# gabrielmittag/NISQA

Hardware: AMD Instinct MI355X
Metric: clips/sec (10 s, 48 kHz) (higher is better)
Workload: dtype bf16x6 (every GEMM -- CNN, projection, self-attention, pooling: fp32 operands as three exact bf16 terms, 6 MFMA products per term pair, f32 accumulate: all 24 operand mantissa bits; mel f32)

## Files before the change

include/nisqa_hip.h:

```cpp
#ifndef NISQA_HIP_H
#define NISQA_HIP_H

#include <stddef.h>
#include <stdint.h>

#ifdef __cplusplus
extern "C" {
#endif

#define NISQA_OK 0
#define NISQA_ERR_ARG 1
#define NISQA_ERR_LAUNCH 2
#define NISQA_ERR_WORKSPACE 3

#define NISQA_ABI_VERSION 2
#define NISQA_N_MELS 48
#define NISQA_SEG_LEN 15
#define NISQA_N_FFT 4096
#define NISQA_FEAT 384
#define NISQA_DMODEL 64

int nisqa_abi_version(void);

typedef struct {
// ... 151 lines not shown
    const uint16_t* pool_wb;
    int32_t arch;
} nisqa_model_dev;

size_t nisqa_workspace_bytes(int32_t n_clips, int32_t total_frames, int32_t total_tok_padded);

int nisqa_predict_batch(const float* pcm, const int64_t* clip_off, const int32_t* frame_off,
                        const int32_t* tok_off, const int32_t* n_wins, int32_t n_clips,
                        int32_t total_frames, int32_t total_tok_padded,
                        const nisqa_mel_cfg* cfg, const nisqa_model_dev* model,
                        void* ws, size_t ws_bytes, float* out, void* stream);

int nisqa_predict_batch_pcm16(const int16_t* pcm, const int64_t* clip_off, const int32_t* frame_off,
                              const int32_t* tok_off, const int32_t* n_wins, int32_t n_clips,
                              int32_t total_frames, int32_t total_tok_padded,
                              const nisqa_mel_cfg* cfg, const nisqa_model_dev* model,
                              void* ws, size_t ws_bytes, float* out, void* stream);

int nisqa_pcm16_to_f32(const int16_t* pcm16, float* pcm, int64_t n, void* stream);

#define NISQA_WAVENC_PCM 1
#define NISQA_WAVENC_FLOAT 3
#define NISQA_WAVENC_ALAW 6
#define NISQA_WAVENC_MULAW 7
#define NISQA_WAVENC_BIG_ENDIAN 0x10000
typedef struct nisqa_wav_clip {
    int64_t src_off;
    int64_t dst_off;
    int64_t n_frames;
    int32_t channels;
    int32_t container;
    int32_t encoding;
    int32_t channel;
} nisqa_wav_clip;
int nisqa_wav_decode(const void* raw, int64_t raw_bytes, const nisqa_wav_clip* clips, int32_t n_clips,
                     int64_t max_frames, float* out, void* stream);

#define NISQA_FLAC_BAD_MD5 0x80
#define NISQA_FLAC_BAD_TABLE 0x100
typedef struct nisqa_flac_clip {
    int64_t src_off;
    int64_t src_bytes;
    int64_t dst_off;
    int64_t n_samples;
    int64_t md5_off;
    int32_t frame0;
    int32_t n_frames;
    int32_t block_size;
    int32_t bits;
    int32_t channels;
    int32_t channel;
    int32_t md5_set;
    int32_t reserved;
    uint8_t md5[16];
} nisqa_flac_clip;
#ifndef NISQA_FLAC_FRAME_DEFINED
#define NISQA_FLAC_FRAME_DEFINED
typedef struct nisqa_flac_frame {
    int32_t offset;
    int32_t first_sample;
    int32_t block_size;
    int32_t clip;
} nisqa_flac_frame;
#endif
size_t nisqa_flac_workspace_bytes(int32_t n_frames, int32_t max_block, int32_t max_channels, int64_t md5_bytes);
int nisqa_flac_decode(const void* raw, int64_t raw_bytes, const nisqa_flac_clip* clips, int32_t n_clips,
                      const nisqa_flac_frame* frames, int32_t n_frames, int32_t max_block, int32_t max_channels,
                      int32_t out_i16, void* out, int64_t out_samples, int64_t md5_bytes, void* ws, size_t ws_bytes,
                      int32_t* status, void* stream);

size_t nisqa_resample_workspace_bytes(int32_t n_clips, int64_t max_out);
int nisqa_resample(const void* pcm, int32_t is_pcm16, const int64_t* in_off, const int64_t* out_off, const int64_t* out_valid,
                   int32_t n_clips, int64_t max_out, double ratio, const float* table, int32_t nwin, int32_t num_table,
                   void* ws, size_t ws_bytes, float* out, void* stream);

int nisqa_de_align_fuse(const float* x, const int32_t* deg_tok_off, const int32_t* deg_n_wins, const int32_t* ref_tok_off,
                        const int32_t* ref_n_wins, int32_t n_pairs, int32_t total_deg_tok_padded, int32_t align, int32_t apply,
                        int32_t fuse, int32_t ld_out, float* out, int32_t* idx_out, void* stream);

int nisqa_selftest_mfma(const float* a, const float* b, float* d, int32_t k, void* stream);

int nisqa_probe_mfma_sustained(const void* operands, float* out, uint64_t* clk, int32_t blocks, int32_t iters, void* stream);

#ifdef __cplusplus
}
#endif
#endif
```

nisqa_amd/csrc/cnn_bf16.hip:

```cpp
#include "common.hpp"
#include "layout.hpp"
#include <stdlib.h>
#include <atomic>
#include "conv_bf16.hpp"
#include "internal.hpp"
#include "../../include/nisqa_hip.h"
#define NQ_RING2 3
#define NQ_RING34 3

#define FB_RS1 48
#define FB_P1 (168 * FB_RS1)
#define FB_RS2 80
#define FB_P2 (60 * FB_RS2)
#define FB_RS3 144
#define FB_P3 (60 * FB_RS3)
#define FB_PS (72 * FB_RS3)
#define FB_PATCH(T) ((T) * FB_P1)
#define FB_PPLANE 1700
#define FB_ZADDR 2048u
#define FB_BASE 2176u
#define FB_WAVE(T) (((T) * (FB_P1 + FB_PPLANE) + 63u) / 64u * 64u)
#define FB_WGS(T) ((T) == 2 ? 2 : 1)
#define FB_LDS(T) (FB_BASE + 4 * FB_WAVE(T))
static_assert(FB_WAVE(2) == 19584 && FB_LDS(2) == 80512 && 2 * FB_LDS(2) <= 160 * 1024, "two terms: two workgroups (8 waves) per CU");
static_assert(FB_WAVE(3) == 29312 && FB_LDS(3) == 119424 && FB_LDS(3) <= 160 * 1024 && 2 * FB_LDS(3) > 160 * 1024, "three terms: one workgroup per CU");
#define FB_PLAN_OK(T) (FB_PATCH(T) + (T) * FB_PPLANE <= FB_WAVE(T) && (T) * FB_P3 <= FB_WAVE(T) && (T) * FB_PS <= 2 * FB_WAVE(T))
static_assert(FB_PLAN_OK(2) && FB_PLAN_OK(3), "LDS plan");

__device__ constexpr int bwin75_lo(int b) { return b == 0 ? 0 : b == 1 ? 1 : b == 2 ? 2 : b == 3 ? 4 : 5; }
__device__ constexpr int bwin75_hi(int b) { return b == 0 ? 2 : b == 1 ? 3 : b == 2 ? 5 : b == 3 ? 6 : 7; }
__device__ constexpr int bwin53_lo(int b) { return b == 0 ? 0 : b == 1 ? 1 : 3; }
__device__ constexpr int bwin53_hi(int b) { return b == 0 ? 2 : b == 1 ? 4 : 5; }

NQ_CLK_EXPORT(g_phase_clk, nisqa_debug_phase_clock)
NQ_CLK_EXPORT(g_phase_clk6, nisqa_debug_phase_clock6)

#define FB_TAB5 0u
#define FB_TAB6 1024u
NQ_DEV f32x2_t lds_ld64(unsigned a) { return *(NQ_AS3 const f32x2_t*)(a); }
template <int FMT>
NQ_DEV float epi_fmt(float v, float c, float t) {
    return FMT == NQ_FMT_BF16X3 || FMT == NQ_FMT_BF16X6 ? fmaxf(v + t, 0.f) : fmaxf(fmaf(v, c, t), 0.f);
}

template <int FMT, int CIN, int MT, int NT, int W, int RS, int PLANE, bool APF, int RING>
NQ_DEV void fb_conv_k(f32x16 (&acc)[MT][NT], __amdgpu_buffer_rsrc_t wrs, int wbyte, unsigned lane16, const unsigned (&base)[MT],
                      const unsigned (&m9)[MT], conv_k_ring<FMT == NQ_FMT_BF16X6 ? 3 : 2, NT, 3>& ring) {
    if constexpr (FMT == NQ_FMT_BF16X6) conv_k_terms_ring<3, CIN, MT, NT, W, RS, PLANE, FB_ZADDR, 3, true, true>(acc, wrs, wbyte, lane16, base, m9, ring);
    else conv_k_bf16<CIN, MT, NT, W, RS, PLANE, FB_ZADDR, APF, RING, FMT>(acc, wrs, wbyte, lane16, base, m9);
}

template <int FMT, bool SEGX, bool P3>
NQ_DEV void cnn_front_split_body(
    const float* __restrict__ mel_tm, const int32_t* __restrict__ frame_off,
    const int32_t* __restrict__ tok_off, const int32_t* __restrict__ n_wins,
    const float* __restrict__ clip_floor, int n_clips, int seg_hop,
    const float* __restrict__ cw, const unsigned short* __restrict__ wb, float* __restrict__ p3,
    float* __restrict__ feat, const float* __restrict__ seg_x, int seg_L,
    const uint32_t* __restrict__ clip_max_enc, float top_db) {
    extern __shared__ __attribute__((aligned(16))) char smem[];
    constexpr bool X6 = FMT == NQ_FMT_BF16X6, F16 = FMT == NQ_FMT_F16X3 || FMT == NQ_FMT_F16X4;
    constexpr int T = X6 ? 3 : 2;
    constexpr bool T16_3 = X6 && (NQ_T16 & 1), T16_4 = X6 && (NQ_T16 & 2);
    constexpr bool CP1 = X6 && (NQ_CPAIR & 1), CP2 = X6 && (NQ_CPAIR & 2);
    static_assert(!P3 || FMT == NQ_FMT_BF16X3, "the fp32 copy of the pooled conv4 tensor is a bf16x3 debug output");
    constexpr int W1_ = X6 ? CNNX_W1 : CNNB_W1, W2_ = X6 ? CNNX_W2 : CNNB_W2, W3_ = X6 ? CNNX_W3 : CNNB_W3, W4_ = X6 ? CNNX_W4 : CNNB_W4,
                  W5_ = X6 ? CNNX_W5 : CNNB_W5, W6_ = X6 ? CNNX_W6 : CNNB_W6, WU16_ = X6 ? CNNX_U16S : CNNB_U16S;
    const int* __restrict__ meta_i = (const int*)(wb + CNNH_META);
    const float* __restrict__ meta_f = (const float*)(wb + CNNH_META);
    float dummy_mx = 0.f;
    NQ_STAMP_BEGIN();
    const int lane = threadIdx.x & 63;
    const int wave = __builtin_amdgcn_readfirstlane(threadIdx.x >> 6);
    const int p0 = blockIdx.x * 4;
    const int b = __builtin_amdgcn_readfirstlane(find_segment_wave(tok_off, n_clips, p0, lane));
    const int k0 = p0 - tok_off[b];
    const int nvalid = min(4, n_wins[b] - k0);
    if (nvalid <= 0) return;
    const bool valid = wave < nvalid;
    const int p = p0 + wave, k = k0 + wave;
    const unsigned R = FB_BASE + wave * FB_WAVE(T);
    const unsigned lane16 = lane * 16;
    const __amdgpu_buffer_rsrc_t wrs = __builtin_amdgcn_make_buffer_rsrc((void*)wb, 0, WU16_ * 2, 0x00020000);
    NQ_STAMP(0);

    const float fl = SEGX ? -3.0e38f : clip_max_enc ? dec_ordered(clip_max_enc[b]) - top_db : clip_floor[b];
    const float* src = SEGX ? seg_x + ((size_t)b * seg_L + k) * 720
                            : mel_tm + (size_t)(frame_off[b] + k * seg_hop) * 48;
    float vraw[12];
#pragma unroll
    for (int q = 0; q < 12; ++q) {
        const int i0 = lane + 64 * q;
        vraw[q] = (valid && (q < 11 || lane < 16)) ? src[i0] : 0.f;
    }
    const float tn1 = cw[CNN_T1 + (lane & 15)], tn2 = cw[CNN_T2 + (lane & 31)];
    const float tn3[2] = {cw[CNN_T3 + (lane & 31)], cw[CNN_T3 + 32 + (lane & 31)]};
    const float tn4[2] = {cw[CNN_T4 + (lane & 31)], cw[CNN_T4 + 32 + (lane & 31)]};
    const float tn5 = cw[CNN_T5 + 16 * wave + (lane & 15)], tn6 = cw[CNN_T6 + 16 * wave + (lane & 15)];
    float vin[12];
#pragma unroll
    for (int q = 0; q < 12; ++q) vin[q] = !valid ? 0.f : SEGX ? vraw[q] : fmaxf(vraw[q], fl);
    int e_in = 0;
    float m_in = 0.f;
    float s0 = 1.f;
    if (F16) {
        float mr = 0.f;
#pragma unroll
        for (int q = 0; q < 12; ++q) mr = fmaxf(mr, __builtin_fabsf(vin[q]));
        m_in = wave_max_nonneg(mr);
        e_in = f16_scale_exp(m_in);
        s0 = pow2_f32(e_in);
    }
    {
        const unsigned pb = R + FB_PATCH(T);
        constexpr int NZ = (T * FB_PPLANE + 15) / 16;
#pragma unroll
        for (int it = 0; it < (NZ + 63) / 64; ++it)
            if (64 * it + 64 <= NZ || lane < NZ - 64 * it) lds_st128(pb + (lane + 64 * it) * 16, f32x4{0.f, 0.f, 0.f, 0.f});
        if (lane < 32) ((unsigned*)(smem + FB_ZADDR))[lane] = 0u;
        __builtin_amdgcn_wave_barrier();
        if (!SEGX) {
            unsigned ob[3];
#pragma unroll
            for (int u = 0; u < 3; ++u) {
                const int e = lane + 16 * u, j0 = e >= 48 ? 1 : 0, m = e - 48 * j0;
                ob[u] = pb + ((j0 + 1) * 50 + m + 1) * 2;
            }
#pragma unroll
            for (int q = 0; q < 12; q += 2) {
                const float v0 = vin[q] * s0, v1 = vin[q + 1] * s0;
                lds_store_pair_fmt<FMT>(ob[q % 3] + (q + q / 3) * 100, ob[(q + 1) % 3] + (q + 1 + (q + 1) / 3) * 100, FB_PPLANE, v0, v1,
                                               dummy_mx, true, q + 1 < 11 || lane < 16);
            }
        } else {
#pragma unroll
            for (int q = 0; q < 12; ++q) {
                const int i0 = lane + 64 * q;
                const int m = i0 / 15, j = i0 - 15 * m;
                if (i0 < 720) lds_store_one_fmt<FMT>(pb + ((j + 1) * 50 + (m + 1)) * 2, FB_PPLANE, vin[q] * s0, dummy_mx);
            }
        }
    }
    __builtin_amdgcn_wave_barrier();
    NQ_STAMP(1);

    const int i = lane & 31, hfi = (i >> 2) & 1, qi = (i & 3) + 4 * (i >> 3);
    const int n = lane & 31, hf = lane >> 5, h = lane >> 5;
    const bool odd = (lane & 1) != 0;

    conv_k_ring<T, 1, 3> ring2;
    if constexpr (X6) conv_k_preload(ring2, wrs, W2_ * 2, lane16);
    {
        f32x4 w1[1][T];
#pragma unroll
        for (int t = 0; t < T; ++t) w1[0][t] = wfrag_load(wrs, lane16, (W1_ + t * 512) * 2);
        float tn = tn1, c1 = 1.f, ms1 = 0.f;
        int e1 = 0;
// ... 396 lines not shown
#pragma unroll
            for (int q = 0; q < T; ++q) b6[g][q] = wfrag_load(wrs, lane16, w6b + (g * T + q) * 1024);
        {
            const unsigned wr = S5 + (4 * kg) * FB_RS3 + ch * 2;
#pragma unroll
            for (int t = 0; t < 5; ++t)
#pragma unroll
                for (int r = 0; r < 4; r += 2)
                    if (t < 4 || kg < 2) {
                        f32x2_t cs0 = {1.f, 1.f}, cs1 = {1.f, 1.f};
                        if (F16) { cs0 = lds_ld64(FB_TAB5 + (16 * t + r) * 8 + kg * 32); cs1 = lds_ld64(FB_TAB5 + (16 * t + r + 1) * 8 + kg * 32); }
                        lds_store_pair_fmt<FMT>(wr + (16 * t + r) * FB_RS3, wr + (16 * t + r + 1) * FB_RS3, FB_PS,
                                                epi_fmt<FMT>(acc5[t][r], cs0[0], tn5 * cs0[1]), epi_fmt<FMT>(acc5[t][r + 1], cs1[0], tn5 * cs1[1]), dummy_mx);
                    }
        }
        __syncthreads();
        NQ_STAMP(10);

        f32x4 acc6[2], acc6b[2];
        unsigned base6[2], m6[2];
#pragma unroll
        for (int t = 0; t < 2; ++t) {
            acc6[t] = f32x4{0.f, 0.f, 0.f, 0.f};
            acc6b[t] = acc6[t];
            const int rho = 16 * t + i16;
            const int slot = rho / 6, y = rho - 6 * slot;
            m6[t] = tap_mask(rho < 24, y, 1, 6, 3);
            base6[t] = S5 + (slot * 18 + (y - 1) * 3) * FB_RS3 + (kg << 4);
        }
        unsigned a6ad[2][T];
        f32x4 a6[2][2][T];
        auto load_a6 = [&](int g) {
            const int tap = g >> 1, s = g & 1;
            const int tapoff = ((tap / 3) * 3 + tap % 3) * FB_RS3;
            if (s == 0) {
#pragma unroll
                for (int t = 0; t < 2; ++t) {
                    const bool ok = (m6[t] >> tap) & 1u;
#pragma unroll
                    for (int q = 0; q < T; ++q) a6ad[t][q] = ok ? base6[t] + q * FB_PS : FB_ZADDR - tapoff;
                }
            }
#pragma unroll
            for (int t = 0; t < 2; ++t)
#pragma unroll
                for (int q = 0; q < T; ++q) a6[g & 1][t][q] = lds_ld128(a6ad[t][q] + tapoff + 64 * s);
        };
        load_a6(0);
#pragma unroll
        for (int g = 0; g < 18; ++g) {
            if (g + 7 < 18) {
#pragma unroll
                for (int q = 0; q < T; ++q) b6[(g + 7) & 7][q] = wfrag_load(wrs, lane16, w6b + ((g + 7) * T + q) * 1024);
            }
            if (g + 1 < 18) load_a6(g + 1);
            f32x4 (&acc)[2] = (g & 1) ? acc6b : acc6;
            if constexpr (X6) {
                __builtin_amdgcn_sched_barrier(0);
                mma16_terms<T, 2>(acc, a6[g & 1], b6[g & 7]);
            } else mma16_pair_fmt<FMT, 2>(acc, a6[g & 1], b6[g & 7]);
        }
        NQ_STAMP(11);
        const unsigned fo = S4 + wave * 2048;
#pragma unroll
        for (int t = 0; t < 2; ++t)
#pragma unroll
            for (int r = 0; r < 4; ++r) {
                const int rho = 16 * t + 4 * kg + r;
                const int slot = rho / 6, y = rho - 6 * slot;
                if (rho < 24) {
                    const float c6 = F16 ? __uint_as_float(lds_ld32(FB_TAB6 + (16 * t + r) * 4 + kg * 16)) : 1.f;
                    lds_st32(fo + (slot * 96 + i16 * 6 + y) * 4, __float_as_uint(epi_fmt<FMT>(acc6[t][r] + acc6b[t][r], c6, tn6)));
                }
            }
        __builtin_amdgcn_wave_barrier();
#pragma unroll
        for (int q0 = 0; q0 < 96; q0 += 64) {
            const int q = q0 + lane;
            const int slot = q / 24;
            if (q < 96 && slot < nvalid)
                *(f32x4*)(feat + (size_t)(p0 + slot) * 384 + 96 * wave + 4 * (q - 24 * slot)) = lds_ld128(fo + 16 * q);
        }
    }
    NQ_STAMP_END((X6 ? g_phase_clk6 : g_phase_clk), ((blockIdx.y * gridDim.x + blockIdx.x) << 2) + wave);
}

#define FB_PARAMS                                                                                                              \
    const float* __restrict__ mel_tm, const int32_t* __restrict__ frame_off, const int32_t* __restrict__ tok_off,             \
    const int32_t* __restrict__ n_wins, const float* __restrict__ clip_floor, int n_clips, int seg_hop,                       \
    const float* __restrict__ cw, const unsigned short* __restrict__ wb, float* __restrict__ p3, float* __restrict__ feat,    \
    const float* __restrict__ seg_x, int seg_L, const uint32_t* __restrict__ clip_max_enc, float top_db
#define FB_ARGS mel_tm, frame_off, tok_off, n_wins, clip_floor, n_clips, seg_hop, cw, wb, p3, feat, seg_x, seg_L, clip_max_enc, top_db
template <bool SEGX, bool P3>
__global__ __launch_bounds__(256, FB_WGS(2)) void cnn_front_bf16_kernel(FB_PARAMS) {
    cnn_front_split_body<NQ_FMT_BF16X3, SEGX, P3>(FB_ARGS);
}
template <bool P4, bool SEGX>
__global__ __launch_bounds__(256, FB_WGS(2)) void cnn_front_f16_kernel(FB_PARAMS) {
    cnn_front_split_body<P4 ? NQ_FMT_F16X4 : NQ_FMT_F16X3, SEGX, false>(FB_ARGS);
}
template <bool SEGX>
__global__ __launch_bounds__(256, FB_WGS(3)) void cnn_front_bf16x6_kernel(FB_PARAMS) {
    cnn_front_split_body<NQ_FMT_BF16X6, SEGX, false>(FB_ARGS);
}

typedef void (*fb_kernel_t)(const float*, const int32_t*, const int32_t*, const int32_t*, const float*, int, int, const float*,
                            const unsigned short*, float*, float*, const float*, int, const uint32_t*, float);
static int fb_launch(int fmt, bool segx, bool p3, const float* mel_tm, const int32_t* frame_off, const int32_t* tok_off,
                     const int32_t* n_wins, const float* clip_floor, const uint32_t* clip_max_enc, float top_db, int32_t n_clips,
                     int32_t total_tok_padded, int32_t seg_hop, const float* cnn_w, const uint16_t* cnn_wb, float* p3_opt, float* feat,
                     const float* seg_x, int32_t seg_L, void* stream) {
    if (n_clips <= 0 || total_tok_padded <= 0 || (total_tok_padded & 31) || seg_hop <= 0 || !cnn_wb || !feat || fmt < 0 || fmt > 3 ||
        (p3 && fmt != 0) || (segx && (!seg_x || seg_L <= 0)) || (!segx && !clip_floor && !clip_max_enc))
        return NISQA_ERR_ARG;
    static const fb_kernel_t kernels[9] = {
        cnn_front_bf16_kernel<false, false>, cnn_front_bf16_kernel<false, true>, cnn_front_bf16_kernel<true, false>,
        cnn_front_f16_kernel<false, false>, cnn_front_f16_kernel<false, true>, cnn_front_f16_kernel<true, false>, cnn_front_f16_kernel<true, true>,
        cnn_front_bf16x6_kernel<false>, cnn_front_bf16x6_kernel<true>};
    const int which = fmt == 0 ? (segx ? 2 : p3 ? 1 : 0) : 3 + 2 * (fmt - 1) + (segx ? 1 : 0);
    const unsigned lds = fmt == NQ_FMT_BF16X6 ? FB_LDS(3) : FB_LDS(2);
    NQ_LAUNCH_BEGIN();
    static std::atomic<bool> lds_ok[9][64];
    if (nq_lds_opt_in((const void*)kernels[which], (int)lds, lds_ok[which])) return 2;
    hipLaunchKernelGGL(kernels[which], dim3(total_tok_padded / 4), dim3(256), lds, (hipStream_t)stream, mel_tm, frame_off, tok_off, n_wins,
                       clip_floor, n_clips, seg_hop, cnn_w, cnn_wb, p3_opt, feat, seg_x, seg_L, clip_max_enc, top_db);
    return NQ_LAUNCH_STATUS();
}

extern "C" int nisqa_cnn_adapt_bf16(const float* mel_tm, const int32_t* frame_off, const int32_t* tok_off,
                                    const int32_t* n_wins, const float* clip_floor, int32_t n_clips,
                                    int32_t total_tok_padded, int32_t seg_hop, const float* cnn_w,
                                    const uint16_t* cnn_wb, float* p3_opt, float* feat, void* stream) {
    if (!clip_floor) return NISQA_ERR_ARG;
    return fb_launch(0, false, p3_opt != nullptr, mel_tm, frame_off, tok_off, n_wins, clip_floor, nullptr, 0.f, n_clips, total_tok_padded, seg_hop,
                     cnn_w, cnn_wb, p3_opt, feat, nullptr, 0, stream);
}

int nq_cnn_adapt_bf16_from_max(const float* mel_tm, const int32_t* frame_off, const int32_t* tok_off,
                               const int32_t* n_wins, const uint32_t* clip_max_enc, float top_db, int32_t n_clips,
                               int32_t total_tok_padded, int32_t seg_hop, const float* cnn_w, const uint16_t* cnn_wb,
                               float* feat, void* stream) {
    if (!clip_max_enc) return NISQA_ERR_ARG;
    return fb_launch(0, false, false, mel_tm, frame_off, tok_off, n_wins, nullptr, clip_max_enc, top_db, n_clips, total_tok_padded, seg_hop, cnn_w,
                     cnn_wb, nullptr, feat, nullptr, 0, stream);
}

extern "C" int nisqa_cnn_adapt_segments_bf16(const float* x, int32_t seg_len_padded, const int32_t* tok_off,
                                             const int32_t* n_wins, int32_t n_clips, int32_t total_tok_padded,
                                             const float* cnn_w, const uint16_t* cnn_wb, float* feat, void* stream) {
    return fb_launch(0, true, false, nullptr, nullptr, tok_off, n_wins, nullptr, nullptr, 0.f, n_clips, total_tok_padded, 1, cnn_w, cnn_wb, nullptr,
                     feat, x, seg_len_padded, stream);
}

extern "C" int nisqa_cnn_adapt_f16(const float* mel_tm, const int32_t* frame_off, const int32_t* tok_off, const int32_t* n_wins,
                                   const float* clip_floor, int32_t n_clips, int32_t total_tok_padded, int32_t seg_hop,
                                   const float* cnn_w, const uint16_t* cnn_wh, int32_t products, float* feat, void* stream) {
    if (!clip_floor || (products != 3 && products != 4)) return NISQA_ERR_ARG;
    return fb_launch(products - 2, false, false, mel_tm, frame_off, tok_off, n_wins, clip_floor, nullptr, 0.f, n_clips, total_tok_padded, seg_hop,
                     cnn_w, cnn_wh, nullptr, feat, nullptr, 0, stream);
}
int nq_cnn_adapt_f16_from_max(const float* mel_tm, const int32_t* frame_off, const int32_t* tok_off, const int32_t* n_wins,
                              const uint32_t* clip_max_enc, float top_db, int32_t n_clips, int32_t total_tok_padded, int32_t seg_hop,
                              const float* cnn_w, const uint16_t* cnn_wh, int32_t products, float* feat, void* stream) {
    if (!clip_max_enc || (products != 3 && products != 4)) return NISQA_ERR_ARG;
    return fb_launch(products - 2, false, false, mel_tm, frame_off, tok_off, n_wins, nullptr, clip_max_enc, top_db, n_clips, total_tok_padded,
                     seg_hop, cnn_w, cnn_wh, nullptr, feat, nullptr, 0, stream);
}
extern "C" int nisqa_cnn_adapt_segments_f16(const float* x, int32_t seg_len_padded, const int32_t* tok_off, const int32_t* n_wins,
                                            int32_t n_clips, int32_t total_tok_padded, const float* cnn_w, const uint16_t* cnn_wh,
                                            int32_t products, float* feat, void* stream) {
    if (products != 3 && products != 4) return NISQA_ERR_ARG;
    return fb_launch(products - 2, true, false, nullptr, nullptr, tok_off, n_wins, nullptr, nullptr, 0.f, n_clips, total_tok_padded, 1, cnn_w, cnn_wh,
                     nullptr, feat, x, seg_len_padded, stream);
}

extern "C" int nisqa_cnn_adapt_bf16x6(const float* mel_tm, const int32_t* frame_off, const int32_t* tok_off,
                                      const int32_t* n_wins, const float* clip_floor, int32_t n_clips,
                                      int32_t total_tok_padded, int32_t seg_hop, const float* cnn_w,
                                      const uint16_t* cnn_wx, float* feat, void* stream) {
    return fb_launch(NQ_FMT_BF16X6, false, false, mel_tm, frame_off, tok_off, n_wins, clip_floor, nullptr, 0.f, n_clips, total_tok_padded, seg_hop,
                     cnn_w, cnn_wx, nullptr, feat, nullptr, 0, stream);
}
int nq_cnn_adapt_bf16x6_from_max(const float* mel_tm, const int32_t* frame_off, const int32_t* tok_off,
                                 const int32_t* n_wins, const uint32_t* clip_max_enc, float top_db, int32_t n_clips,
                                 int32_t total_tok_padded, int32_t seg_hop, const float* cnn_w, const uint16_t* cnn_wx,
                                 float* feat, void* stream) {
    if (!clip_max_enc) return NISQA_ERR_ARG;
    return fb_launch(NQ_FMT_BF16X6, false, false, mel_tm, frame_off, tok_off, n_wins, nullptr, clip_max_enc, top_db, n_clips, total_tok_padded,
                     seg_hop, cnn_w, cnn_wx, nullptr, feat, nullptr, 0, stream);
}
extern "C" int nisqa_cnn_adapt_segments_bf16x6(const float* x, int32_t seg_len_padded, const int32_t* tok_off,
                                               const int32_t* n_wins, int32_t n_clips, int32_t total_tok_padded,
                                               const float* cnn_w, const uint16_t* cnn_wx, float* feat, void* stream) {
    return fb_launch(NQ_FMT_BF16X6, true, false, nullptr, nullptr, tok_off, n_wins, nullptr, nullptr, 0.f, n_clips, total_tok_padded, 1, cnn_w, cnn_wx,
                     nullptr, feat, x, seg_len_padded, stream);
}
```

nisqa_amd/csrc/internal.hpp:

```cpp
#pragma once
#include <stdint.h>

int nq_cnn_adapt_bf16_from_max(const float* mel_tm, const int32_t* frame_off, const int32_t* tok_off,
                               const int32_t* n_wins, const uint32_t* clip_max_enc, float top_db, int32_t n_clips,
                               int32_t total_tok_padded, int32_t seg_hop, const float* cnn_w, const uint16_t* cnn_wb,
                               float* feat, void* stream);

int nq_cnn_adapt_f16_from_max(const float* mel_tm, const int32_t* frame_off, const int32_t* tok_off, const int32_t* n_wins,
                              const uint32_t* clip_max_enc, float top_db, int32_t n_clips, int32_t total_tok_padded, int32_t seg_hop,
                              const float* cnn_w, const uint16_t* cnn_wh, int32_t products, float* feat, void* stream);

int nq_cnn_adapt_bf16x6_from_max(const float* mel_tm, const int32_t* frame_off, const int32_t* tok_off,
                                 const int32_t* n_wins, const uint32_t* clip_max_enc, float top_db, int32_t n_clips,
                                 int32_t total_tok_padded, int32_t seg_hop, const float* cnn_w, const uint16_t* cnn_wx,
                                 float* feat, void* stream);
```

nisqa_amd/lib.py:

```python
import ctypes
import os

_HERE = os.path.dirname(os.path.abspath(__file__))
LIB_PATH = os.environ.get('NISQA_HIP_LIB') or os.path.join(_HERE, 'libnisqa_hip.so')

NISQA_OK, NISQA_ERR_ARG, NISQA_ERR_LAUNCH, NISQA_ERR_WORKSPACE = 0, 1, 2, 3
ABI_VERSION = 2
LSTM_POOL_LAST_STEP_BI, LSTM_POOL_AVG, LSTM_POOL_MAX = 0, 1, 2

c_p = ctypes.c_void_p
c_i32 = ctypes.c_int32
c_i64 = ctypes.c_int64


class MelCfg(ctypes.Structure):
    _fields_ = [('n_fft', c_i32), ('hop', c_i32), ('win', c_i32), ('n_mels', c_i32), ('n_bins', c_i32),
                ('w_floats', c_i32), ('amin_sq', ctypes.c_float), ('top_db', ctypes.c_float)]


class ModelDev(ctypes.Structure):
    _fields_ = [('window', c_p), ('twiddle', c_p), ('band_start', c_p), ('band_len', c_p), ('band_woff', c_p),
                ('band_w', c_p), ('cnn_w', c_p), ('td_w', c_p), ('pool_w', c_p),
                ('n_layers', c_i32), ('n_heads', c_i32), ('seg_hop', c_i32), ('stage_events', c_p),
                ('cnn_wb', c_p), ('cnn_mode', c_i32), ('td_wb', c_p), ('pool_wb', c_p), ('arch', c_i32)]


class WavClip(ctypes.Structure):
    _fields_ = [('src_off', c_i64), ('dst_off', c_i64), ('n_frames', c_i64), ('channels', c_i32), ('container', c_i32),
                ('encoding', c_i32), ('channel', c_i32)]


class FlacClip(ctypes.Structure):
    _fields_ = [('src_off', c_i64), ('src_bytes', c_i64), ('dst_off', c_i64), ('n_samples', c_i64), ('md5_off', c_i64),
                ('frame0', c_i32), ('n_frames', c_i32), ('block_size', c_i32), ('bits', c_i32), ('channels', c_i32),
                ('channel', c_i32), ('md5_set', c_i32), ('reserved', c_i32), ('md5', ctypes.c_uint8 * 16)]


class FlacFrame(ctypes.Structure):
    _fields_ = [('offset', c_i32), ('first_sample', c_i32), ('block_size', c_i32), ('clip', c_i32)]


FLAC_BAD_MD5, FLAC_BAD_TABLE = 0x80, 0x100
WAVENC_PCM, WAVENC_FLOAT, WAVENC_ALAW, WAVENC_MULAW, WAVENC_BIG_ENDIAN = 1, 3, 6, 7, 0x10000
MEL_GATHER_LDS_CLIPS = 1024
WAV_DECODE_MAX_BLOCK, WAV_DECODE_MAX_MEAN = 1024, 32

SYMBOLS = {
    'nisqa_abi_version': (ctypes.c_int, []),
    'nisqa_mel_db': (ctypes.c_int, [c_p, c_p, c_p, c_i32, c_i32, ctypes.POINTER(MelCfg), c_p, c_p, c_p, c_p, c_p, c_p,
                                    c_p, c_p, c_p]),
    'nisqa_mel_db_pcm16': (ctypes.c_int, [c_p, c_p, c_p, c_i32, c_i32, ctypes.POINTER(MelCfg), c_p, c_p, c_p, c_p, c_p, c_p,
                                          c_p, c_p, c_p]),
    'nisqa_mel_finalize': (ctypes.c_int, [c_p, c_p, c_i32, c_i32, c_p, ctypes.c_float, c_p, c_i32, c_p]),
    'nisqa_cnn_adapt': (ctypes.c_int, [c_p, c_p, c_p, c_p, c_p, c_i32, c_i32, c_i32, c_p, c_p, c_p, c_p]),
    'nisqa_cnn_front': (ctypes.c_int, [c_p, c_p, c_p, c_p, c_p, c_i32, c_i32, c_i32, c_p, c_p, c_p]),
    'nisqa_cnn_adapt_bf16': (ctypes.c_int, [c_p, c_p, c_p, c_p, c_p, c_i32, c_i32, c_i32, c_p, c_p, c_p, c_p, c_p]),
    'nisqa_cnn_adapt_segments_bf16': (ctypes.c_int, [c_p, c_i32, c_p, c_p, c_i32, c_i32, c_p, c_p, c_p, c_p]),
    'nisqa_cnn_adapt_bf16x6': (ctypes.c_int, [c_p, c_p, c_p, c_p, c_p, c_i32, c_i32, c_i32, c_p, c_p, c_p, c_p]),
    'nisqa_cnn_adapt_segments_bf16x6': (ctypes.c_int, [c_p, c_i32, c_p, c_p, c_i32, c_i32, c_p, c_p, c_p, c_p]),
    'nisqa_cnn_adapt_f16': (ctypes.c_int, [c_p, c_p, c_p, c_p, c_p, c_i32, c_i32, c_i32, c_p, c_p, c_i32, c_p, c_p]),
    'nisqa_cnn_adapt_segments_f16': (ctypes.c_int, [c_p, c_i32, c_p, c_p, c_i32, c_i32, c_p, c_p, c_i32, c_p, c_p]),
    'nisqa_cnn_adapt_segments': (ctypes.c_int, [c_p, c_i32, c_p, c_p, c_i32, c_i32, c_p, c_p, c_p, c_p]),
    'nisqa_cnn_back': (ctypes.c_int, [c_p, c_p, c_p, c_i32, c_i32, c_p, c_p, c_p]),
    'nisqa_cnn_standard': (ctypes.c_int, [c_p, c_p, c_p, c_p, c_p, c_i32, c_i32, c_i32, c_p, c_p, c_p, c_p]),
    'nisqa_cnn_standard_bf16': (ctypes.c_int, [c_p, c_p, c_p, c_p, c_p, c_i32, c_i32, c_i32, c_p, c_p, c_p, c_p]),
    'nisqa_cnn_standard_bf16x6': (ctypes.c_int, [c_p, c_p, c_p, c_p, c_p, c_i32, c_i32, c_i32, c_p, c_p, c_p, c_p]),
    'nisqa_cnn_standard_f16': (ctypes.c_int, [c_p, c_p, c_p, c_p, c_p, c_i32, c_i32, c_i32, c_p, c_p, c_i32, c_p, c_p]),
    'nisqa_cnn_standard_segments': (ctypes.c_int, [c_p, c_i32, c_p, c_p, c_i32, c_i32, c_p, c_p, c_p, c_p]),
    'nisqa_cnn_standard_segments_bf16': (ctypes.c_int, [c_p, c_i32, c_p, c_p, c_i32, c_i32, c_p, c_p, c_p, c_p]),
    'nisqa_cnn_standard_segments_bf16x6': (ctypes.c_int, [c_p, c_i32, c_p, c_p, c_i32, c_i32, c_p, c_p, c_p, c_p]),
    'nisqa_cnn_standard_segments_f16': (ctypes.c_int, [c_p, c_i32, c_p, c_p, c_i32, c_i32, c_p, c_p, c_i32, c_p, c_p]),
    'nisqa_lstm_laststep': (ctypes.c_int, [c_p, c_p, c_p, c_i32, c_p, c_p, c_p, c_p, c_p]),
    'nisqa_lstm_pool': (ctypes.c_int, [c_p, c_p, c_p, c_i32, c_p, c_i32, c_p, c_p, c_p, c_p]),
    'nisqa_td_selfatt': (ctypes.c_int, [c_p, c_p, c_p, c_i32, c_i32, c_i32, c_p, c_p, c_p, c_p]),
    'nisqa_td_selfatt_bf16': (ctypes.c_int, [c_p, c_p, c_p, c_i32, c_i32, c_i32, c_p, c_p, c_p, c_p, c_p]),
    'nisqa_pool_att_bf16': (ctypes.c_int, [c_p, c_p, c_p, c_i32, c_i32, c_i32, c_p, c_p, c_p, c_p, c_p]),
    'nisqa_td_selfatt_bf16x6': (ctypes.c_int, [c_p, c_p, c_p, c_i32, c_i32, c_i32, c_p, c_p, c_p, c_p, c_p]),
    'nisqa_pool_att_bf16x6': (ctypes.c_int, [c_p, c_p, c_p, c_i32, c_i32, c_i32, c_p, c_p, c_p, c_p, c_p]),
    'nisqa_td_pool_bf16x6': (ctypes.c_int, [c_p, c_p, c_p, c_i32, c_i32, c_i32, c_p, c_p, c_i32, c_p, c_p, c_p, c_p, c_p, c_p]),
    'nisqa_pool_score_bf16': (ctypes.c_int, [c_p, c_p, c_p, c_i32, c_i32, c_i32, c_p, c_p, c_p, c_p]),
    'nisqa_pool_score_bf16x6': (ctypes.c_int, [c_p, c_p, c_p, c_i32, c_i32, c_i32, c_p, c_p, c_p, c_p]),
    'nisqa_pool_final': (ctypes.c_int, [c_p, c_p, c_i32, c_i32, c_i32, c_p, c_p, c_p]),
    'nisqa_pool_att': (ctypes.c_int, [c_p, c_p, c_p, c_i32, c_i32, c_i32, c_p, c_p, c_p, c_p]),
    'nisqa_pool_profile': (ctypes.c_int, [c_p, c_i32, c_p, c_p, c_i32, c_i32, c_i32, c_i32, c_p, c_p, c_p, c_p]),
    'nisqa_pool_profile_bwd': (ctypes.c_int, [c_p, c_i32, c_p, c_p, c_i32, c_i32, c_i32, c_i32, c_p, c_p, c_p, c_p, c_p, c_p]),
    'nisqa_workspace_bytes': (ctypes.c_size_t, [c_i32, c_i32, c_i32]),
    'nisqa_predict_batch': (ctypes.c_int, [c_p, c_p, c_p, c_p, c_p, c_i32, c_i32, c_i32, ctypes.POINTER(MelCfg),
                                           ctypes.POINTER(ModelDev), c_p, ctypes.c_size_t, c_p, c_p]),
    'nisqa_predict_batch_pcm16': (ctypes.c_int, [c_p, c_p, c_p, c_p, c_p, c_i32, c_i32, c_i32, ctypes.POINTER(MelCfg),
                                                 ctypes.POINTER(ModelDev), c_p, ctypes.c_size_t, c_p, c_p]),
    'nisqa_pcm16_to_f32': (ctypes.c_int, [c_p, c_p, c_i64, c_p]),
    'nisqa_wav_decode': (ctypes.c_int, [c_p, c_i64, c_p, c_i32, c_i64, c_p, c_p]),
    'nisqa_flac_workspace_bytes': (ctypes.c_size_t, [c_i32, c_i32, c_i32, c_i64]),
    'nisqa_flac_decode': (ctypes.c_int, [c_p, c_i64, c_p, c_i32, c_p, c_i32, c_i32, c_i32, c_i32, c_p, c_i64, c_i64, c_p,
                                         ctypes.c_size_t, c_p, c_p]),
    'nisqa_resample_workspace_bytes': (ctypes.c_size_t, [c_i32, c_i64]),
    'nisqa_resample': (ctypes.c_int, [c_p, c_i32, c_p, c_p, c_p, c_i32, c_i64, ctypes.c_double, c_p, c_i32, c_i32, c_p, ctypes.c_size_t, c_p, c_p]),
    'nisqa_de_align_fuse': (ctypes.c_int, [c_p, c_p, c_p, c_p, c_p, c_i32, c_i32, c_i32, c_i32, c_i32, c_i32, c_p, c_p, c_p]),
    'nisqa_selftest_mfma': (ctypes.c_int, [c_p, c_p, c_p, c_i32, c_p]),
    'nisqa_probe_mfma_sustained': (ctypes.c_int, [c_p, c_p, c_p, c_i32, c_i32, c_p]),
}

class TdTrainArgs(ctypes.Structure):
    _fields_ = [('n_clips', c_i32), ('n_tokens', c_i32), ('n_tokens_padded', c_i32), ('n_layers', c_i32), ('n_heads', c_i32),
                ('n_wgrad_groups', c_i32), ('n_wgrad_tiles', c_i32), ('n_colsum_jobs', c_i32),
                ('seg_off', c_p), ('ptok_off', c_p), ('tile_clip', c_p), ('sq_off', c_p), ('params', c_p), ('grads', c_p),
                ('poff', c_p), ('ws', c_p), ('frags', c_p), ('labels', c_p), ('bias_map', c_p), ('inv_count', c_p),
                ('mask_p', c_p * 4), ('mask_1', c_p * 4), ('mask_f', c_p * 4), ('mask_2', c_p * 4),
                ('wgrad_desc', c_p), ('colsum_jobs', c_p)]


c_f = ctypes.c_float
TRAIN_SYMBOLS = {
    'nisqa_tdtrain_plan': (ctypes.c_int, [c_i32, c_i32, c_i32, c_i32, c_i32, c_p, c_p, c_i64]),
    'nisqa_tdtrain_step': (ctypes.c_int, [ctypes.POINTER(TdTrainArgs), c_p]),
    'nisqa_tdtrain_step_heads': (ctypes.c_int, [ctypes.POINTER(TdTrainArgs), c_p]),
    'nisqa_gemm_f32': (ctypes.c_int, [c_p, c_p, c_p, c_p, c_i32, c_i32, c_i32, c_i32, c_i32, c_f, c_p]),
    'nisqa_gemm_f32_one': (ctypes.c_int, [c_p, c_p, c_p, c_i64, c_i64, c_i64, c_i64, c_i64, c_i64, c_i32, c_i32, c_i32,
                                          c_f, c_p, c_i32, c_p]),
    'nisqa_gemm_f32_one_tile': (ctypes.c_int, [c_i64, c_i64, ctypes.POINTER(c_i32), ctypes.POINTER(c_i32)]),
    'nisqa_conv1_fwd': (ctypes.c_int, [c_p, c_p, c_p, c_p, c_i32, c_i32, c_i32, c_p, c_p, c_p, c_p]),
    'nisqa_conv1_wgrad': (ctypes.c_int, [c_p, c_p, c_p, c_p, c_i32, c_i32, c_i32, c_p, c_p, c_p]),
    'nisqa_conv1_moments': (ctypes.c_int, [c_p, c_p, c_p, c_p, c_i32, c_i32, c_i32, c_p, c_p]),
    'nisqa_conv1_bn_act_pool_fwd': (ctypes.c_int, [c_p] * 4 + [c_i32] * 3 + [c_p] * 13),
    'nisqa_conv1_bn_act_pool_bwd': (ctypes.c_int, [c_p] * 4 + [c_i32] * 3 + [c_p] * 14),
    'nisqa_im2col_mel': (ctypes.c_int, [c_p, c_p, c_p, c_p, c_i32, c_i32, c_i32, c_p, c_p]),
    'nisqa_conv1_bn_act_pool_std_fwd': (ctypes.c_int, [c_p] * 4 + [c_i32] * 3 + [c_p] * 13),
    'nisqa_conv1_bn_act_pool_std_bwd': (ctypes.c_int, [c_p] * 4 + [c_i32] * 3 + [c_p] * 14),
    'nisqa_lstm_train_fwd': (ctypes.c_int, [c_p, c_p, c_i32, c_p, c_p, c_p, c_p, c_i32, c_p, c_p, c_p, c_p, c_p]),
    'nisqa_lstm_train_bptt': (ctypes.c_int, [c_p, c_i32, c_p, c_p, c_i32, c_p, c_p, c_p, c_p, c_p]),
    'nisqa_im2col3x3': (ctypes.c_int, [c_p, c_i32, c_i32, c_i32, c_i32, c_i32, c_p, c_p]),
    'nisqa_conv3x3_gemm': (ctypes.c_int, [c_i32, c_p, c_p, c_p, c_i32, c_i32, c_i32, c_i32, c_i32, c_i32, c_p, c_i32, c_p]),
    'nisqa_conv3x3_fwd_stats': (ctypes.c_int, [c_i32, c_p, c_p, c_p, c_i32, c_i32, c_i32, c_i32, c_i32, c_i32, c_p, c_p, c_p]),
    'nisqa_conv3x3_gemm_bf16': (ctypes.c_int, [c_i32, c_p, c_p, c_p, c_i32, c_i32, c_i32, c_i32, c_i32, c_i32, c_p, c_i32, c_p]),
    'nisqa_segconv_supported': (ctypes.c_int, [c_i32, c_i32, c_i32, c_i32, c_i32]),
    'nisqa_segconv_frag_bytes': (ctypes.c_int64, [c_i32, c_i32, c_i32]),
    'nisqa_segconv_pack': (ctypes.c_int, [c_i32, c_p, c_i32, c_i32, c_p, c_p]),
    'nisqa_segconv_pack_many': (ctypes.c_int, [c_i32, c_p, c_p, c_p, c_p, c_p, c_p]),
    'nisqa_segconv_bf16': (ctypes.c_int, [c_i32, c_p, c_p, c_p, c_i32, c_i32, c_i32, c_i32, c_i32, c_i32, c_p, c_p, c_p]),
    'nisqa_segconv_frag_bytes_f32': (ctypes.c_int64, [c_i32, c_i32, c_i32]),
    'nisqa_segconv_pack_f32_many': (ctypes.c_int, [c_i32, c_p, c_p, c_p, c_p, c_p, c_p]),
    'nisqa_segconv_f32': (ctypes.c_int, [c_i32, c_p, c_p, c_p, c_i32, c_i32, c_i32, c_i32, c_i32, c_i32, c_p, c_p, c_p]),
    'nisqa_segconv_frag_bytes_x6': (ctypes.c_int64, [c_i32, c_i32, c_i32]),
    'nisqa_segconv_frag_bytes_f16': (ctypes.c_int64, [c_i32, c_i32, c_i32]),
    'nisqa_segconv_pack_f16_many': (ctypes.c_int, [c_i32, c_p, c_p, c_p, c_p, c_p, c_p]),
    'nisqa_segconv_f16': (ctypes.c_int, [c_i32, c_p, c_p, c_p, c_i32, c_i32, c_i32, c_i32, c_i32, c_i32, c_p, c_p, c_p]),
    'nisqa_segconv_pack_x6_many': (ctypes.c_int, [c_i32, c_p, c_p, c_p, c_p, c_p, c_p]),
    'nisqa_segconv_bf16x6': (ctypes.c_int, [c_i32, c_p, c_p, c_p, c_i32, c_i32, c_i32, c_i32, c_i32, c_i32, c_p, c_p, c_p]),
    'nisqa_segconv_wgrad_bf16': (ctypes.c_int, [c_p, c_p, c_p, c_i32, c_i32, c_i32, c_i32, c_i32, c_i32, c_p]),
    'nisqa_col2im3x3': (ctypes.c_int, [c_p, c_i32, c_i32, c_i32, c_i32, c_i32, c_p, c_p]),
    'nisqa_col_dot': (ctypes.c_int, [c_p, c_p, c_i64, c_i32, c_p, c_p]),
    'nisqa_bn_act_pool_fwd': (ctypes.c_int, [c_p, c_p, c_p, c_p, c_p, c_p, c_p, c_i32, c_i32, c_i32, c_i32, c_i32, c_i32,
                                             c_p, c_p, c_p, c_p]),
    'nisqa_bn_act_pool_bwd1': (ctypes.c_int, [c_p, c_p, c_p, c_p, c_p, c_p, c_p, c_i32, c_i32, c_i32, c_i32, c_i32, c_i32,
                                              c_p, c_p, c_p]),
    'nisqa_bn_act_pool_bwd': (ctypes.c_int, [c_p] * 7 + [c_i32] * 6 + [c_p] * 5),
    'nisqa_bn_pool_bwd_sums': (ctypes.c_int, [c_p] * 7 + [c_i32] * 6 + [c_p] * 2),
    'nisqa_segconv_wgrad_bn_bf16': (ctypes.c_int, [c_p] * 13 + [c_i32] * 8 + [c_p]),
    'nisqa_segconv_wgrad_f32': (ctypes.c_int, [c_p] * 13 + [c_i32] * 8 + [c_p]),
    'nisqa_segconv_wgrad_bf16x6': (ctypes.c_int, [c_p] * 13 + [c_i32] * 8 + [c_p]),
    'nisqa_bn_bwd2': (ctypes.c_int, [c_p, c_p, c_p, c_p, c_p, c_i64, c_i32, c_p, c_p, c_p, c_p]),
    'nisqa_layernorm_fwd': (ctypes.c_int, [c_p, c_p, c_p, c_i64, c_p, c_p, c_p, c_p]),
    'nisqa_layernorm_bwd': (ctypes.c_int, [c_p, c_p, c_p, c_p, c_i64, c_p, c_p]),
    'nisqa_softmax_rows_fwd': (ctypes.c_int, [c_p, c_p, c_p, c_i64, c_f, c_p, c_p]),
    'nisqa_softmax_rows_bwd': (ctypes.c_int, [c_p, c_p, c_p, c_p, c_i64, c_f, c_p, c_p]),
    'nisqa_elementwise': (ctypes.c_int, [c_i32, c_p, c_p, c_p, c_i64, c_i32, c_p, c_p]),
    'nisqa_mse_loss': (ctypes.c_int, [c_p, c_p, c_p, c_i32, c_i32, c_p, c_p, c_p]),
    'nisqa_mse_loss_heads': (ctypes.c_int, [c_p, c_p, c_p, c_i32, c_i32, c_p, c_p, c_p]),
    'nisqa_dropout_mask': (ctypes.c_int, [ctypes.c_uint64, ctypes.c_uint64, c_f, c_i64, c_p, c_p]),
    'nisqa_cast_scatter': (ctypes.c_int, [c_p, c_p, c_i32, c_p, c_p]),
    'nisqa_adam_step': (ctypes.c_int, [c_p, c_p, c_p, c_p, c_i64, c_f, c_i32, c_p]),
    'nisqa_de_align_fuse_packed': (ctypes.c_int, [c_p] * 6 + [c_i32] * 5 + [c_p] * 3),
    'nisqa_de_align_fuse_bwd': (ctypes.c_int, [c_p, c_i32] + [c_p] * 5 + [c_i32] * 3 + [c_p] * 3),
    'nisqa_de_align_soft_packed': (ctypes.c_int, [c_p] * 6 + [c_i32] * 5 + [c_p] * 4),
    'nisqa_de_align_soft_bwd': (ctypes.c_int, [c_p, c_p, c_i32] + [c_p] * 6 + [c_i32] * 4 + [c_p] * 3),
    'nisqa_mel_gather': (ctypes.c_int, [c_p, c_i64, c_p, c_p, c_i32, c_p, c_p, c_i32, c_i32, c_p, c_p, c_p]),
    'nisqa_bn_eval_act_pool_fwd': (ctypes.c_int, [c_p] * 5 + [c_i32] * 6 + [c_p] * 3),
    'nisqa_bn_eval_act_pool_bwd': (ctypes.c_int, [c_p] * 7 + [c_i32] * 6 + [c_p] * 2),
    'nisqa_conv1_segments_fwd': (ctypes.c_int, [c_p, c_i32, c_p, c_i32, c_i32, c_p, c_p, c_p, c_p]),
    'nisqa_conv1_segments_dgrad': (ctypes.c_int, [c_p, c_p, c_i32, c_i32, c_p, c_p, c_p]),
    'nisqa_bn_eval_act_maxpool2_fwd': (ctypes.c_int, [c_p] * 5 + [c_i32] * 5 + [c_p] * 3),
    'nisqa_bn_eval_act_maxpool2_bwd': (ctypes.c_int, [c_p] * 7 + [c_i32] * 5 + [c_p] * 2),
    'nisqa_segments_to_mel_bwd': (ctypes.c_int, [c_p, c_i32, c_p, c_p, c_i32, c_i32, c_i32, c_p, c_p]),
# ... 124 lines not shown
```

Measured before the change: 63690.

## Run bf16x6 CNN front end as a persistent grid with rotated item assignment

The bf16x6 CNN front-end kernel, which fits only one workgroup per CU, now launches a persistent grid sized to resident capacity when there are more items than slots. Each workgroup loops over items with a coprime rotation stride, so later waves of work are spread across CUs. This removes per-workgroup launch and tail costs and the large-LDS workgroup turnover. The loop version is built in a separate translation unit, and a host API caps the grid size. The risks are extra __syncthreads and loop overhead, possible load imbalance, and register pressure from the looping body.

```diff
diff --git a/include/nisqa_hip.h b/include/nisqa_hip.h
--- a/include/nisqa_hip.h
+++ b/include/nisqa_hip.h
@@ -257,6 +257,8 @@
 
 int nisqa_probe_mfma_sustained(const void* operands, float* out, uint64_t* clk, int32_t blocks, int32_t iters, void* stream);
 
+void nisqa_cnn_loop_set_max_workgroups(int32_t n);
+
 #ifdef __cplusplus
 }
 #endif
diff --git a/nisqa_amd/csrc/cnn_bf16.hip b/nisqa_amd/csrc/cnn_bf16.hip
--- a/nisqa_amd/csrc/cnn_bf16.hip
+++ b/nisqa_amd/csrc/cnn_bf16.hip
@@ -1,6 +1,7 @@
 #include "common.hpp"
 #include "layout.hpp"
 #include <stdlib.h>
+#include <algorithm>
 #include <atomic>
 #include "conv_bf16.hpp"
 #include "internal.hpp"
@@ -32,8 +33,13 @@
 __device__ constexpr int bwin53_lo(int b) { return b == 0 ? 0 : b == 1 ? 1 : 3; }
 __device__ constexpr int bwin53_hi(int b) { return b == 0 ? 2 : b == 1 ? 4 : 5; }
 
+#ifdef FB_LOOP_UNIT
+NQ_CLK_EXPORT(g_phase_clk6, nisqa_debug_phase_clock6)
+#define FB_CLK g_phase_clk6
+#else
 NQ_CLK_EXPORT(g_phase_clk, nisqa_debug_phase_clock)
-NQ_CLK_EXPORT(g_phase_clk6, nisqa_debug_phase_clock6)
+#define FB_CLK g_phase_clk
+#endif
 
 #define FB_TAB5 0u
 #define FB_TAB6 1024u
@@ -50,14 +56,14 @@
     else conv_k_bf16<CIN, MT, NT, W, RS, PLANE, FB_ZADDR, APF, RING, FMT>(acc, wrs, wbyte, lane16, base, m9);
 }
 
-template <int FMT, bool SEGX, bool P3>
-NQ_DEV void cnn_front_split_body(
+template <int FMT, bool SEGX, bool P3, bool LOOP>
+NQ_DEV void cnn_front_split_item(
     const float* __restrict__ mel_tm, const int32_t* __restrict__ frame_off,
     const int32_t* __restrict__ tok_off, const int32_t* __restrict__ n_wins,
     const float* __restrict__ clip_floor, int n_clips, int seg_hop,
     const float* __restrict__ cw, const unsigned short* __restrict__ wb, float* __restrict__ p3,
     float* __restrict__ feat, const float* __restrict__ seg_x, int seg_L,
-    const uint32_t* __restrict__ clip_max_enc, float top_db) {
+    const uint32_t* __restrict__ clip_max_enc, float top_db, const int item) {
     extern __shared__ __attribute__((aligned(16))) char smem[];
     constexpr bool X6 = FMT == NQ_FMT_BF16X6, F16 = FMT == NQ_FMT_F16X3 || FMT == NQ_FMT_F16X4;
     constexpr int T = X6 ? 3 : 2;
@@ -70,9 +76,13 @@
     const float* __restrict__ meta_f = (const float*)(wb + CNNH_META);
     float dummy_mx = 0.f;
     NQ_STAMP_BEGIN();
-    const int lane = threadIdx.x & 63;
-    const int wave = __builtin_amdgcn_readfirstlane(threadIdx.x >> 6);
-    const int p0 = blockIdx.x * 4;
+    int lane = threadIdx.x & 63, wave_v = threadIdx.x >> 6;
+    if constexpr (LOOP) {
+        asm volatile("" : "+v"(lane), "+v"(wave_v));
+        __builtin_assume(lane >= 0 && lane < 64);
+    }
+    const int wave = __builtin_amdgcn_readfirstlane(wave_v);
+    const int p0 = item * 4;
     const int b = __builtin_amdgcn_readfirstlane(find_segment_wave(tok_off, n_clips, p0, lane));
     const int k0 = p0 - tok_off[b];
     const int nvalid = min(4, n_wins[b] - k0);
@@ -635,7 +645,7 @@
                 *(f32x4*)(feat + (size_t)(p0 + slot) * 384 + 96 * wave + 4 * (q - 24 * slot)) = lds_ld128(fo + 16 * q);
         }
     }
-    NQ_STAMP_END((X6 ? g_phase_clk6 : g_phase_clk), ((blockIdx.y * gridDim.x + blockIdx.x) << 2) + wave);
+    NQ_STAMP_END(FB_CLK, (item << 2) + wave);
 }
 
 #define FB_PARAMS                                                                                                              \
@@ -644,17 +654,36 @@
     const float* __restrict__ cw, const unsigned short* __restrict__ wb, float* __restrict__ p3, float* __restrict__ feat,    \
     const float* __restrict__ seg_x, int seg_L, const uint32_t* __restrict__ clip_max_enc, float top_db
 #define FB_ARGS mel_tm, frame_off, tok_off, n_wins, clip_floor, n_clips, seg_hop, cw, wb, p3, feat, seg_x, seg_L, clip_max_enc, top_db
+template <int FMT, bool SEGX, bool P3, bool LOOP>
+NQ_DEV void cnn_front_split_body(FB_PARAMS, int n_items, int rot) {
+    static_assert(!LOOP || FMT == NQ_FMT_BF16X6, "only the one-workgroup-per-CU format loops");
+    if constexpr (!LOOP) {
+        cnn_front_split_item<FMT, SEGX, P3, false>(FB_ARGS, blockIdx.x);
+    } else {
+        const int G = gridDim.x;
+        int pos = blockIdx.x;
+        for (int item0 = 0; item0 + pos < n_items; item0 += G) {
+            cnn_front_split_item<FMT, SEGX, P3, true>(FB_ARGS, item0 + pos);
+            pos += rot;
+            pos -= pos >= G ? G : 0;
+            __syncthreads();
+        }
+    }
+}
+
+#ifndef FB_LOOP_UNIT
 template <bool SEGX, bool P3>
 __global__ __launch_bounds__(256, FB_WGS(2)) void cnn_front_bf16_kernel(FB_PARAMS) {
-    cnn_front_split_body<NQ_FMT_BF16X3, SEGX, P3>(FB_ARGS);
+    cnn_front_split_body<NQ_FMT_BF16X3, SEGX, P3, false>(FB_ARGS, 0, 0);
 }
 template <bool P4, bool SEGX>
 __global__ __launch_bounds__(256, FB_WGS(2)) void cnn_front_f16_kernel(FB_PARAMS) {
-    cnn_front_split_body<P4 ? NQ_FMT_F16X4 : NQ_FMT_F16X3, SEGX, false>(FB_ARGS);
-}
+    cnn_front_split_body<P4 ? NQ_FMT_F16X4 : NQ_FMT_F16X3, SEGX, false, false>(FB_ARGS, 0, 0);
+}
+
 template <bool SEGX>
-__global__ __launch_bounds__(256, FB_WGS(3)) void cnn_front_bf16x6_kernel(FB_PARAMS) {
-    cnn_front_split_body<NQ_FMT_BF16X6, SEGX, false>(FB_ARGS);
+__global__ __launch_bounds__(256, FB_WGS(3)) void cnn_front_bf16x6_item_kernel(FB_PARAMS) {
+    cnn_front_split_body<NQ_FMT_BF16X6, SEGX, false, false>(FB_ARGS, 0, 0);
 }
 
 typedef void (*fb_kernel_t)(const float*, const int32_t*, const int32_t*, const int32_t*, const float*, int, int, const float*,
@@ -666,20 +695,87 @@
     if (n_clips <= 0 || total_tok_padded <= 0 || (total_tok_padded & 31) || seg_hop <= 0 || !cnn_wb || !feat || fmt < 0 || fmt > 3 ||
         (p3 && fmt != 0) || (segx && (!seg_x || seg_L <= 0)) || (!segx && !clip_floor && !clip_max_enc))
         return NISQA_ERR_ARG;
+    const int items = total_tok_padded / 4;
+    if (fmt == NQ_FMT_BF16X6) {
+        const int G = nq_cnn_front_bf16x6_grid(segx, items);
+        if (G <= 0) return 2;
+        if (G < items)
+            return nq_cnn_front_bf16x6_launch(segx, G, mel_tm, frame_off, tok_off, n_wins, clip_floor, clip_max_enc, top_db, n_clips, items, seg_hop,
+                                              cnn_w, cnn_wb, feat, seg_x, seg_L, stream);
+    }
     static const fb_kernel_t kernels[9] = {
         cnn_front_bf16_kernel<false, false>, cnn_front_bf16_kernel<false, true>, cnn_front_bf16_kernel<true, false>,
         cnn_front_f16_kernel<false, false>, cnn_front_f16_kernel<false, true>, cnn_front_f16_kernel<true, false>, cnn_front_f16_kernel<true, true>,
-        cnn_front_bf16x6_kernel<false>, cnn_front_bf16x6_kernel<true>};
+        cnn_front_bf16x6_item_kernel<false>, cnn_front_bf16x6_item_kernel<true>};
     const int which = fmt == 0 ? (segx ? 2 : p3 ? 1 : 0) : 3 + 2 * (fmt - 1) + (segx ? 1 : 0);
     const unsigned lds = fmt == NQ_FMT_BF16X6 ? FB_LDS(3) : FB_LDS(2);
     NQ_LAUNCH_BEGIN();
     static std::atomic<bool> lds_ok[9][64];
     if (nq_lds_opt_in((const void*)kernels[which], (int)lds, lds_ok[which])) return 2;
-    hipLaunchKernelGGL(kernels[which], dim3(total_tok_padded / 4), dim3(256), lds, (hipStream_t)stream, mel_tm, frame_off, tok_off, n_wins,
+    hipLaunchKernelGGL(kernels[which], dim3(items), dim3(256), lds, (hipStream_t)stream, mel_tm, frame_off, tok_off, n_wins,
                        clip_floor, n_clips, seg_hop, cnn_w, cnn_wb, p3_opt, feat, seg_x, seg_L, clip_max_enc, top_db);
     return NQ_LAUNCH_STATUS();
 }
 
+#else
+template <bool SEGX>
+__global__ __launch_bounds__(256, FB_WGS(3)) void cnn_front_bf16x6_kernel(FB_PARAMS, int n_items, int rot) {
+    cnn_front_split_body<NQ_FMT_BF16X6, SEGX, false, true>(FB_ARGS, n_items, rot);
+}
+typedef void (*fb_loop_kernel_t)(const float*, const int32_t*, const int32_t*, const int32_t*, const float*, int, int, const float*,
+                                 const unsigned short*, float*, float*, const float*, int, const uint32_t*, float, int, int);
+
+static std::atomic<int> fb_loop_max_wgs{0};
+extern "C" void nisqa_cnn_loop_set_max_workgroups(int32_t n) { fb_loop_max_wgs.store(n > 0 ? n : 0, std::memory_order_relaxed); }
+
+static int fb_loop_resident(const void* kernel, unsigned lds, std::atomic<int> (&cache)[64]) {
+    int dev = 0;
+    if (hipGetDevice(&dev) != hipSuccess || dev < 0 || dev >= 64) dev = 0;
+    int r = cache[dev].load(std::memory_order_relaxed);
+    if (r <= 0) {
+        int per_cu = 0, cus = 0;
+        if (hipOccupancyMaxActiveBlocksPerMultiprocessor(&per_cu, kernel, 256, lds) != hipSuccess ||
+            hipDeviceGetAttribute(&cus, hipDeviceAttributeMultiprocessorCount, dev) != hipSuccess || per_cu <= 0 || cus <= 0)
+            return 0;
+        r = per_cu * cus;
+        cache[dev].store(r, std::memory_order_relaxed);
+    }
+    return r;
+}
+static int fb_loop_rot(int G) {
+    if (G < 3) return G - 1;
+    auto gcd = [](int a, int b) { while (b) { const int t = a % b; a = b; b = t; } return a; };
+    int c = (int)((long long)G * 618 / 1000);
+    if (c < 1) c = 1;
+    while (gcd(c, G) != 1) ++c;
+    return c;
+}
+
+static const fb_loop_kernel_t fb_loop_kernels[2] = {cnn_front_bf16x6_kernel<false>, cnn_front_bf16x6_kernel<true>};
+static std::atomic<bool> fb_loop_lds_ok[2][64];
+int nq_cnn_front_bf16x6_grid(bool segx, int32_t items) {
+    const int which = segx ? 1 : 0;
+    static std::atomic<int> resident[2][64];
+    if (nq_lds_opt_in((const void*)fb_loop_kernels[which], (int)FB_LDS(3), fb_loop_lds_ok[which])) return 0;
+    const int res = fb_loop_resident((const void*)fb_loop_kernels[which], FB_LDS(3), resident[which]);
+    if (res <= 0) return 0;
+    const int cap = fb_loop_max_wgs.load(std::memory_order_relaxed);
+    return std::min((int)items, cap > 0 ? std::min(cap, res) : res);
+}
+int nq_cnn_front_bf16x6_launch(bool segx, int32_t G, const float* mel_tm, const int32_t* frame_off, const int32_t* tok_off, const int32_t* n_wins,
+                               const float* clip_floor, const uint32_t* clip_max_enc, float top_db, int32_t n_clips, int32_t items,
+                               int32_t seg_hop, const float* cnn_w, const uint16_t* cnn_wb, float* feat, const float* seg_x, int32_t seg_L,
+                               void* stream) {
+    const int which = segx ? 1 : 0;
+    NQ_LAUNCH_BEGIN();
+    if (G <= 0 || nq_lds_opt_in((const void*)fb_loop_kernels[which], (int)FB_LDS(3), fb_loop_lds_ok[which])) return 2;
+    hipLaunchKernelGGL(fb_loop_kernels[which], dim3(G), dim3(256), FB_LDS(3), (hipStream_t)stream, mel_tm, frame_off, tok_off, n_wins, clip_floor,
+                       n_clips, seg_hop, cnn_w, cnn_wb, (float*)nullptr, feat, seg_x, seg_L, clip_max_enc, top_db, items, fb_loop_rot(G));
+    return NQ_LAUNCH_STATUS();
+}
+#endif
+
+#ifndef FB_LOOP_UNIT
 extern "C" int nisqa_cnn_adapt_bf16(const float* mel_tm, const int32_t* frame_off, const int32_t* tok_off,
                                     const int32_t* n_wins, const float* clip_floor, int32_t n_clips,
                                     int32_t total_tok_padded, int32_t seg_hop, const float* cnn_w,
@@ -748,3 +844,4 @@
     return fb_launch(NQ_FMT_BF16X6, true, false, nullptr, nullptr, tok_off, n_wins, nullptr, nullptr, 0.f, n_clips, total_tok_padded, 1, cnn_w, cnn_wx,
                      nullptr, feat, x, seg_len_padded, stream);
 }
+#endif
diff --git a/nisqa_amd/csrc/cnn_bf16x6.hip b/nisqa_amd/csrc/cnn_bf16x6.hip
--- /dev/null
+++ b/nisqa_amd/csrc/cnn_bf16x6.hip
@@ -0,0 +1,2 @@
+#define FB_LOOP_UNIT
+#include "cnn_bf16.hip"
diff --git a/nisqa_amd/csrc/internal.hpp b/nisqa_amd/csrc/internal.hpp
--- a/nisqa_amd/csrc/internal.hpp
+++ b/nisqa_amd/csrc/internal.hpp
@@ -14,3 +14,9 @@
                                  const int32_t* n_wins, const uint32_t* clip_max_enc, float top_db, int32_t n_clips,
                                  int32_t total_tok_padded, int32_t seg_hop, const float* cnn_w, const uint16_t* cnn_wx,
                                  float* feat, void* stream);
+
+int nq_cnn_front_bf16x6_grid(bool segx, int32_t items);
+int nq_cnn_front_bf16x6_launch(bool segx, int32_t G, const float* mel_tm, const int32_t* frame_off, const int32_t* tok_off, const int32_t* n_wins,
+                               const float* clip_floor, const uint32_t* clip_max_enc, float top_db, int32_t n_clips, int32_t items,
+                               int32_t seg_hop, const float* cnn_w, const uint16_t* cnn_wb, float* feat, const float* seg_x, int32_t seg_L,
+                               void* stream);
diff --git a/nisqa_amd/lib.py b/nisqa_amd/lib.py
--- a/nisqa_amd/lib.py
+++ b/nisqa_amd/lib.py
@@ -99,6 +99,7 @@
     'nisqa_de_align_fuse': (ctypes.c_int, [c_p, c_p, c_p, c_p, c_p, c_i32, c_i32, c_i32, c_i32, c_i32, c_i32, c_p, c_p, c_p]),
     'nisqa_selftest_mfma': (ctypes.c_int, [c_p, c_p, c_p, c_i32, c_p]),
     'nisqa_probe_mfma_sustained': (ctypes.c_int, [c_p, c_p, c_p, c_i32, c_i32, c_p]),
+    'nisqa_cnn_loop_set_max_workgroups': (None, [c_i32]),
 }
 
 class TdTrainArgs(ctypes.Structure):
```

Measured after the change: 64070 (median of 6 runs). No clear change (+0.6%).
